# rccohn/AMPIS

Measured on AMD Instinct MI355X. Metric: images/sec Mask R-CNN R50-FPN @1024x1024 inference, higher is better.
Workload: dtype f32 (convs: f16x3 split-operand MFMA -- 22-bit operands, exact products, fp32 accumulate); 1 GPU; BASELINE configs[1]: R50-FPN inference, batch=8 synthetic 1024x1024 micrographs per GPU, K=2, 1000 proposals/img, TEST.DETECTIONS_PER_IMAGE=200, seeded random-init weights, outputs on the host: boxes, scores, classes and every mask as its COCO compressed-RLE counts string (encoded on the device); batch_per_gpu=8, global_batch=8, parallelism=image-parallel replicas x1, no data-path collective

## Files before the change

### ampis_amd/_lib.py

```python
import ctypes as C
import os

_HERE = os.path.dirname(os.path.abspath(__file__))
LIB_PATH = os.path.join(_HERE, "lib", "libampis_hip.so")


class AmpError(RuntimeError):
    pass


class ConvDesc(C.Structure):
    _fields_ = [(n, C.c_int) for n in
                ("B", "H", "W", "Cin", "Cout", "KH", "KW", "stride", "pad", "relu", "res_mode", "out_mode")]


class RpnLevels(C.Structure):
    _fields_ = [("nlevels", C.c_int), ("A", C.c_int), ("ld", C.c_int), ("pred", C.c_void_p * 5),
                ("h", C.c_int * 5), ("w", C.c_int * 5), ("stride", C.c_int * 5), ("anchor_size", C.c_int * 5)]


class FpnFeats(C.Structure):
    _fields_ = [("feat", C.c_void_p * 4), ("h", C.c_int * 4), ("w", C.c_int * 4), ("stride", C.c_int * 4),
                ("C", C.c_int)]

# ... 56 lines not shown

def _declare(L):
    vp, i, f = C.c_void_p, C.c_int, C.c_float
    sig = {
        "amp_version": ([], i),
        "amp_init": ([i, vp, i, C.POINTER(vp)], i),
        "amp_timer_start": ([vp], i),
        "amp_prof_begin": ([vp, i], i),
        "amp_prof_end": ([vp, C.POINTER(ProfSummary)], i),
        "amp_prof_pause": ([vp, i], i),
        "amp_prof_launches": ([vp, C.POINTER(ProfLaunch), i, C.POINTER(i)], i),
        "amp_timer_stop": ([vp, C.POINTER(f)], i),
        "amp_destroy": ([vp], None),
        "amp_sync": ([vp], i),
        "amp_malloc": ([vp, C.c_size_t, C.POINTER(vp)], i),
        "amp_free": ([vp, vp], i),
        "amp_memcpy_h2d": ([vp, vp, vp, C.c_size_t], i),
        "amp_memcpy_d2h": ([vp, vp, vp, C.c_size_t], i),
        "amp_memset": ([vp, vp, i, C.c_size_t], i),
        "amp_conv2d_nhwc": ([vp, C.POINTER(ConvDesc), vp, vp, vp, vp, vp, vp], i),
        "amp_conv2d_nhwc_ex": ([vp, C.POINTER(ConvDesc), vp, vp, vp, vp, vp, vp, vp], i),
        "amp_conv2d_nhwc_fmt": ([vp, C.POINTER(ConvDesc), vp, vp, vp, vp, vp, vp, i], i),
        "amp_unsplit_rows": ([vp, vp, C.c_longlong, i, vp], i),
        "amp_group_expand_weights": ([vp, vp, i, i, i, i, vp], i),
        "amp_resize_scratch_bytes": ([i, i, i, i], C.c_size_t),
        "amp_resize_bilinear_u8": ([vp, vp, i, i, vp, i, i, vp], i),
        "amp_resize_flip_u8": ([vp, vp, i, i, vp, i, i, i, i, vp], i),
        "amp_compact_dets": ([vp, i, i, vp, vp, vp, vp, vp, vp, vp, vp], i),
        "amp_set_conv_mode": ([vp, i], i),
        "amp_get_conv_mode": ([vp], i),
        "amp_conv_range_flag": ([vp, i, C.POINTER(C.c_int)], i),
        "amp_split_weights": ([vp, vp, C.c_longlong, i, vp], i),
        "amp_bottleneck64_tail": ([vp, i, i, i, vp, vp, vp, vp, vp, vp, vp, i, vp, vp], i),
        "amp_conv2d_grouped_nhwc": ([vp, C.POINTER(ConvDesc), i, vp, vp, vp, vp, vp, vp], i),
        "amp_conv2d_grouped_nhwc_fmt": ([vp, C.POINTER(ConvDesc), i, vp, vp, vp, vp, vp, vp, i], i),
        "amp_conv_wgrad_scratch_floats": ([C.POINTER(ConvDesc)], C.c_size_t),
        "amp_conv2d_wgrad": ([vp, C.POINTER(ConvDesc), vp, vp, vp, vp, vp, i], i),
        "amp_conv2d_wgrad_scaled": ([vp, C.POINTER(ConvDesc), vp, vp, vp, vp, vp, i, i, i], i),
        "amp_colsum": ([vp, vp, i, i, vp, vp, i], i),
        "amp_dgrad_weights": ([vp, vp, vp, i, i, i, i, vp], i),
        "amp_dgrad_weights_split": ([vp, vp, vp, i, i, i, i, vp], i),
        "amp_preprocess": ([vp, vp, i, i, i, i, i, C.POINTER(f), C.POINTER(f), vp, vp], i),
        "amp_model_set_image_sizes": ([vp, vp, i], i),
        "amp_maxpool3x3s2": ([vp, vp, i, i, i, i, vp], i),
        "amp_subsample2": ([vp, vp, i, i, i, i, vp], i),
        "amp_rpn_topk": ([vp, C.POINTER(RpnLevels), i, i, vp, i, vp, vp, vp], i),
        "amp_rpn_decode": ([vp, C.POINTER(RpnLevels), i, i, vp, vp, vp, i, i, i, vp, vp, vp], i),
        "amp_rpn_decode_sized": ([vp, C.POINTER(RpnLevels), i, i, vp, vp, vp, i, i, vp, i, vp, vp, vp], i),
        "amp_sort_gather": ([vp, i, i, i, vp, vp, vp, vp, vp, vp, vp, vp, vp], i),
        "amp_sort_gather_n": ([vp, i, i, i, vp, vp, vp, vp, vp, vp, vp, vp, vp, vp], i),
        "amp_nms": ([vp, i, i, vp, vp, vp, f, i, vp, vp, vp], i),
        "amp_rpn_nms_scratch_words": ([i, i, i], C.c_size_t),
        "amp_rpn_nms_levels": ([vp, i, i, i, i, vp, vp, vp, f, i, vp, vp, vp, vp, vp, vp, vp], i),
        "amp_roi_align": ([vp, C.POINTER(FpnFeats), vp, vp, vp, i, i, vp, vp], i),
        "amp_roi_align_fmt": ([vp, C.POINTER(FpnFeats), vp, vp, vp, i, i, vp, vp, i], i),
        "amp_box_candidates": ([vp, vp, i, vp, vp, i, i, i, C.POINTER(f), f, i, i, vp, vp, i, vp, vp], i),
        "amp_box_candidates_sized": ([vp, vp, i, vp, vp, i, i, i, C.POINTER(f), f, i, i, vp, vp, vp, i, vp, vp], i),
        "amp_gather_dets": ([vp, i, i, i, vp, vp, vp, vp, vp, vp, vp, vp, vp, vp], i),
        "amp_mask_prob": ([vp, vp, vp, i, i, vp], i),
        "amp_mask_deconv_predict": ([vp, vp, i, vp, vp, vp, vp, vp, i, vp], i),
        "amp_paste_rle": ([vp, vp, vp, vp, i, vp, vp, i, i, i, f, vp, vp, vp, C.c_ulonglong, vp, vp, vp, vp], i),
        "amp_paste_rle_sized": ([vp, vp, vp, vp, i, vp, vp, i, i, i, vp, f, vp, vp, vp, C.c_ulonglong, vp, vp, vp, vp, vp, C.c_ulonglong, vp], i),
        "amp_rle_to_string": ([vp, i, vp, C.c_size_t, C.POINTER(C.c_size_t)], i),
        "amp_rle_to_strings": ([vp, vp, vp, i, vp, C.c_size_t, vp], i),
        "amp_rle_from_string": ([vp, C.c_size_t, vp, i, C.POINTER(i)], i),
        "amp_rle_encode": ([vp, i, i, vp, i, C.POINTER(i)], i),
# ... 229 lines not shown
```

### ampis_amd/csrc/common.h

```cpp
#pragma once
#include <hip/hip_runtime.h>
#ifdef __HIPCC__
#include <hip/hip_ext.h>
#endif
#include <stdint.h>
#include <stdio.h>
#include <algorithm>
#include <string>

#include "../../include/ampis_hip.h"

namespace amp {

void set_error(const char* fmt, ...);

#define AMP_HIP_CHECK(expr)                                                         \
    do {                                                                            \
        hipError_t _e = (expr);                                                     \
        if (_e != hipSuccess) {                                                     \
            amp::set_error("%s:%d: %s -> %s", __FILE__, __LINE__, #expr,            \
                           hipGetErrorString(_e));                                  \
            return AMP_ERR_HIP;                                                     \
        }                                                                           \
    } while (0)
// ... 140 lines not shown
int comm_mark_producer_end(amp_ctx* ctx);
int comm_wait_done(amp_ctx* ctx);
int comm_agree_flag(amp_ctx* ctx, int* d_flag);
int rle_strings_run(amp_ctx* ctx, const unsigned int* pool, const unsigned long long* off, const int* len, int n, char* str,
                    unsigned long long cap, unsigned long long* str_off, int* str_len, unsigned long long* total);
int roi_align_run(amp_ctx* ctx, const amp_fpn_feats* f, const float* rois, const int* batch_idx, const int* roi_count, int R, int P,
                  float* out, int* level_out, int out_split, int in_split = 0);
int box_candidates_run(amp_ctx* ctx, const float* pred, int ld, const float* proposals, const int* prop_count, int B, int Rcap, int K,
                       const float reg_weights[4], float score_thresh, int img_h, int img_w, const int* img_hw, const float* thresh_img,
                       float* dense_boxes, unsigned long long* keys, int ccap, int* cand_count, int* overflow);
struct WeightJob {
    const float* w;
    const float* scale;
    unsigned int* out;
    int N, KH, KW, C;
    int transpose;
};
int weight_jobs_run(amp_ctx* ctx, const WeightJob* jobs_dev, const void* chunks_dev, int nchunks);
int sgd_chunks_run(amp_ctx* ctx, const unsigned long long* chunks_dev, int nchunks, float* p, const float* g, float* v, float lr,
                   float momentum, float weight_decay, float grad_scale);
int wgrad_async_begin(amp_ctx* ctx, float* scratch1);
int wgrad_async_join(amp_ctx* ctx);
int wgrad_async_end(amp_ctx* ctx);
int roi_align_bwd_run(amp_ctx* ctx, float* const dfeat[4], const int fh[4], const int fw[4], const int stride[4], int C, const float* rois,
                      const int* batch_idx, int R, int P, const float* dout, int B, int init);
int upsample2_bwd_run(amp_ctx* ctx, const float* dfine, float* dcoarse, int B, int Hc, int Wc, int C, int init);
int maxpool_run(amp_ctx* ctx, const float* x, int B, int H, int W, int C, float* y, int y_split);
int compact_dets_run(amp_ctx* ctx, int B, int D, const int* det_count, const float* det_boxes, const float* det_scores, const int* det_classes,
                     float* boxes, float* scores, int* classes, int* batch, int* n_total );
int stem_pool_run(amp_ctx* ctx, int B, int H, int W, const float* x, int x_split, const float* w_split, const float* scale, const float* shift,
                  float* pool, int pool_split);
int conv_c64_fused3_run(amp_ctx* ctx, int B, int H, int W, const float* x_split, const float* w2_split, const float* scale2, const float* shift2,
                        const float* w3_split, const float* scale3, const float* shift3, int C3, const float* res_split, float* y_split);
bool stem_pool_applies(amp_ctx* ctx, const float* w_split);
bool stem_u8_applies(amp_ctx* ctx, const float* w_split);
int stem_pool_u8_run(amp_ctx* ctx, const uint8_t* img, int B, int H, int W, int Hp, int Wp, const float mean[3], const float std_[3],
                     const int* img_hw, const float* w_split, const float* scale, const float* shift, float* pool, int pool_split);
int preprocess_run(amp_ctx* ctx, const uint8_t* img_bgr, int B, int H, int W, int Hp, int Wp, const float mean[3], const float std[3],
                   const int* img_hw, float* out, int out_split);
}
```

### ampis_amd/csrc/conv.hip

```cpp
#include "common.h"
#include <type_traits>

namespace {

typedef float f32x4 __attribute__((ext_vector_type(4)));
typedef float f32x16 __attribute__((ext_vector_type(16)));
typedef _Float16 f16x8 __attribute__((ext_vector_type(8)));
typedef _Float16 f16x2 __attribute__((ext_vector_type(2)));
typedef _Float16 f16x4 __attribute__((ext_vector_type(4)));
typedef unsigned int u32x4 __attribute__((ext_vector_type(4)));
constexpr float LO_SCALE = 2048.0f;

constexpr int BK = 32;
constexpr int LDS_LD = 36;

struct ConvArgs {
    const float* x;
    const float* w;
    const float* scale;
    const float* shift;
    const float* res;
    const float* mask;
    float* y;
    int B, H, W, Cin;
// ... 1903 lines not shown
    const int oyw = oy0 + 4 * wm;
    if constexpr (EPI == 3) {
        const int Ho = a.Ho, Wo = a.Wo, M = a.M;
        conv_epilogue_rpn_rows(a, acc, lds, wave, lane, n0, [=](int i, int r) {
            const int oy = oyw + i, ox = ox0 + r;
            return (oy < Ho && ox < Wo) ? (b * Ho + oy) * Wo + ox : M;
        });
    } else {
#pragma unroll
        for (int h = 0; h < 2; ++h) {
            int mrows[2];
#pragma unroll
            for (int i = 0; i < 2; ++i) {
                const int oy = oyw + 2 * h + i, ox = ox0 + l15;
                mrows[i] = (oy < a.Ho && ox < a.Wo) ? (b * a.Ho + oy) * a.Wo + ox : a.M;
            }
            conv_epilogue_direct_rows<false, true, 2>(a, reinterpret_cast<f32x4 (&)[2][4]>(acc[2 * h]), lane, mrows, n0 + wn * 64);
        }
    }
#ifdef AMP_STAMP
    if (lane == 0)
        for (int q = 0; q < 8; ++q) atomicAdd(&g_stamp[wave * 8 + q], (unsigned long long)st_acc[q]);
#endif
}

struct Fuse3Args {
    const float* w3;
    const float* scale3;
    const float* shift3;
    const float* res;
    float* y;
    int C3;
    unsigned int w3_bytes;
};
template <bool DIAG, bool FUSE3 = false>
__global__ __launch_bounds__(256, 2) void conv3x3_c64_kernel(const ConvArgs a, const unsigned int x_bytes, const unsigned int w_bytes, const int tiles_x, const int tiles_y, const Fuse3Args f3) {
    constexpr int TH = 8, TW = 16, PH = TH + 2, PW = TW + 2, NPIX = PH * PW;
    constexpr int ROWF = 64;
    constexpr int NINST = NPIX / 4;
    static_assert(NPIX % 4 == 0, "patch pixels per DMA instruction");
    __shared__ __attribute__((aligned(16))) float lds[NPIX * ROWF + 2 * 64 * ROWF];
    float* patch = lds;
    float* wbuf = lds + NPIX * ROWF;
    const int tid = threadIdx.x, lane = tid & 63;
    const int wave = __builtin_amdgcn_readfirstlane(tid >> 6);
    const int l15 = lane & 15, lq = lane >> 4;
    int t = amp::xcd_remap(blockIdx.x, a.nblk);
    const int tile_n = t % a.ntn; t /= a.ntn;
    const int tx = t % tiles_x; t /= tiles_x;
    const int ty = t % tiles_y;
    const int b = t / tiles_y;
    const int oy0 = ty * TH, ox0 = tx * TW, n0 = tile_n * 64;
    const int cwin = a.grouped ? n0 : 0;
    const __amdgpu_buffer_rsrc_t rsrc_x = __builtin_amdgcn_make_buffer_rsrc(const_cast<float*>(a.x), 0, x_bytes, 0x00020000);
    const __amdgpu_buffer_rsrc_t rsrc_w = __builtin_amdgcn_make_buffer_rsrc(const_cast<float*>(a.w), 0, w_bytes, 0x00020000);
    const int sub = lane >> 4, chunk = lane & 15;
    for (int it = wave; it < NINST; it += 4) {
        const int q = it * 4 + sub;
        const int py = q / PW, px = q - py * PW;
        const int iy = oy0 - 1 + py, ix = ox0 - 1 + px;
        const bool v = (unsigned)iy < (unsigned)a.H && (unsigned)ix < (unsigned)a.W;
        const unsigned int voff = v ? (unsigned int)((((size_t)(b * a.H + iy) * a.W + ix) * a.Cin + cwin) * 4 + (size_t)((chunk ^ (q & 15)) * 16)) : OOB_VOFF;
        __builtin_amdgcn_raw_ptr_buffer_load_lds(rsrc_x, (__attribute__((address_space(3))) void*)(patch + it * 4 * ROWF), 16, (int)voff, 0, 0, 0);
    }
    auto stage_w = [&](int tap, int buf) {
#pragma unroll
        for (int g = 0; g < 4; ++g) {
            const int r = (wave * 4 + g) * 4 + sub;
            const int n = n0 + swap_channel(r);
            const unsigned int voff = (n < a.Cout) ? (unsigned int)(((size_t)n * a.K + (size_t)tap * 64) * 4 + (size_t)((chunk ^ (r & 15)) * 16)) : OOB_VOFF;
            __builtin_amdgcn_raw_ptr_buffer_load_lds(rsrc_w, (__attribute__((address_space(3))) void*)(wbuf + buf * 64 * ROWF + (wave * 4 + g) * 4 * ROWF), 16, (int)voff, 0, 0, 0);
        }
    };
    stage_w(0, 0);
    f32x4 acc[2][4], acx[2][4];
#pragma unroll
    for (int i = 0; i < 2; ++i)
#pragma unroll
        for (int j = 0; j < 4; ++j)
#pragma unroll
            for (int e = 0; e < 4; ++e) { acc[i][j][e] = 0.f; acx[i][j][e] = 0.f; }
    for (int tap = 0; tap < 9; ++tap) {
        __syncthreads();
        if (tap + 1 < 9) stage_w(tap + 1, (tap + 1) & 1);
        const int ky = tap / 3, kx = tap - 3 * ky;
        const float* wb = wbuf + (tap & 1) * 64 * ROWF;
#pragma unroll
        for (int g = 0; g < 2; ++g) {
            F16x3Frags<2, 4> f;
#pragma unroll
            for (int i = 0; i < 2; ++i) {
                const int q = (2 * wave + i + ky) * PW + kx + l15;
                const float* row = patch + q * ROWF;
                f.ah[i] = *reinterpret_cast<const f16x8*>(row + 4 * ((8 * g + lq) ^ (q & 15)));
                f.al[i] = *reinterpret_cast<const f16x8*>(row + 4 * ((8 * g + 4 + lq) ^ (q & 15)));
            }
            if constexpr (DIAG) {
#pragma unroll
                for (int jj = 0; jj < 2; ++jj) {
                    const float* row = wb + ((2 * g + jj) * 16 + l15) * ROWF;
                    f.bh[jj] = *reinterpret_cast<const f16x8*>(row + 4 * ((8 * g + lq) ^ l15));
                    f.bl[jj] = *reinterpret_cast<const f16x8*>(row + 4 * ((8 * g + 4 + lq) ^ l15));
                }
#pragma unroll
                for (int i = 0; i < 2; ++i) {
#pragma unroll
                    for (int jj = 0; jj < 2; ++jj) acx[i][2 * g + jj] = __builtin_amdgcn_mfma_f32_16x16x32_f16(f.bh[jj], f.al[i], acx[i][2 * g + jj], 0, 0, 0);
#pragma unroll
                    for (int jj = 0; jj < 2; ++jj) acx[i][2 * g + jj] = __builtin_amdgcn_mfma_f32_16x16x32_f16(f.bl[jj], f.ah[i], acx[i][2 * g + jj], 0, 0, 0);
#pragma unroll
                    for (int jj = 0; jj < 2; ++jj) acc[i][2 * g + jj] = __builtin_amdgcn_mfma_f32_16x16x32_f16(f.bh[jj], f.ah[i], acc[i][2 * g + jj], 0, 0, 0);
                }
            } else {
#pragma unroll
                for (int j = 0; j < 4; ++j) {
                    const float* row = wb + (j * 16 + l15) * ROWF;
                    f.bh[j] = *reinterpret_cast<const f16x8*>(row + 4 * ((8 * g + lq) ^ l15));
                    f.bl[j] = *reinterpret_cast<const f16x8*>(row + 4 * ((8 * g + 4 + lq) ^ l15));
                }
                f16x3_mfma16<2, 4, true>(f, acc, acx);
            }
        }
    }
#pragma unroll
    for (int i = 0; i < 2; ++i)
#pragma unroll
        for (int j = 0; j < 4; ++j)
#pragma unroll
            for (int e = 0; e < 4; ++e) acc[i][j][e] = __fadd_rn(acc[i][j][e], __fmul_rn(acx[i][j][e], 1.0f / LO_SCALE));
    int mrows[2];
#pragma unroll
    for (int i = 0; i < 2; ++i) {
        const int oy = oy0 + 2 * wave + i, ox = ox0 + l15;
        mrows[i] = (oy < a.Ho && ox < a.Wo) ? (b * a.Ho + oy) * a.Wo + ox : a.M;
    }
    if constexpr (!FUSE3) {
        conv_epilogue_direct_rows<false, true, 2>(a, acc, lane, mrows, n0);
    } else {
        f16x8 t2h[2][2], t2l[2][2];
        f32x2 chk = {0.f, 0.f};
#pragma unroll
        for (int g = 0; g < 2; ++g) {
            f32x2 sc[4], sh[4];
            const int n = 32 * g + 8 * lq;
#pragma unroll
            for (int p = 0; p < 4; ++p) {
                sc[p] = a.scale ? f32x2{a.scale[n + 2 * p], a.scale[n + 2 * p + 1]} : f32x2{1.f, 1.f};
                sh[p] = a.shift ? f32x2{a.shift[n + 2 * p], a.shift[n + 2 * p + 1]} : f32x2{0.f, 0.f};
            }
#pragma unroll
            for (int i = 0; i < 2; ++i) {
#pragma unroll
                for (int p = 0; p < 4; ++p) {
                    const f32x4& blk = acc[i][2 * g + (p >> 1)];
                    const f32x2 v = {blk[2 * (p & 1)], blk[2 * (p & 1) + 1]};
                    chk = __builtin_elementwise_fma(v, f32x2{0.f, 0.f}, chk);
                    f32x2 o = v * sc[p] + sh[p];
                    if (a.relu) { o[0] = fmaxf(o[0], 0.f); o[1] = fmaxf(o[1], 0.f); }
                    const f16x2 h = __builtin_convertvector(o, f16x2);
                    const f32x2 hf = {(float)h[0], (float)h[1]};
                    const f32x2 l = __builtin_elementwise_fma(hf, f32x2{-LO_SCALE, -LO_SCALE}, o * LO_SCALE);
                    const f16x2 lh = __builtin_convertvector(l, f16x2);
                    t2h[i][g][2 * p] = h[0]; t2h[i][g][2 * p + 1] = h[1];
                    t2l[i][g][2 * p] = lh[0]; t2l[i][g][2 * p + 1] = lh[1];
                }
            }
        }
        if (!(chk[0] == 0.f) || !(chk[1] == 0.f)) atomicOr(a.range_flag, 1);
        __syncthreads();
        const __amdgpu_buffer_rsrc_t rsrc_w3 = __builtin_amdgcn_make_buffer_rsrc(const_cast<float*>(f3.w3), 0, f3.w3_bytes, 0x00020000);
        float* w3s = lds;
        const int ninst3 = f3.C3 / 4;
        for (int it = wave; it < ninst3; it += 4) {
            const int r = it * 4 + sub;
            const int n = (r & ~63) + swap_channel(r & 63);
            const unsigned int voff = (unsigned int)((size_t)n * 256 + (size_t)((chunk ^ (r & 15)) * 16));
            __builtin_amdgcn_raw_ptr_buffer_load_lds(rsrc_w3, (__attribute__((address_space(3))) void*)(w3s + it * 4 * ROWF), 16, (int)voff, 0, 0, 0);
        }
        __syncthreads();
        ConvArgs a3 = a;
        a3.scale = f3.scale3; a3.shift = f3.shift3; a3.res = f3.res; a3.mask = nullptr; a3.y = f3.y;
        a3.Cout = f3.C3; a3.relu = 1; a3.res_mode = 1; a3.res_split = 1; a3.y_split = 1; a3.out_mode = 0; a3.mask_split = 0;
        for (int c = 0; c < f3.C3 / 64; ++c) {
            f32x4 acc3[2][4], acx3[2][4];
#pragma unroll
            for (int i = 0; i < 2; ++i)
#pragma unroll
                for (int j = 0; j < 4; ++j)
#pragma unroll
                    for (int e = 0; e < 4; ++e) { acc3[i][j][e] = 0.f; acx3[i][j][e] = 0.f; }
            const float* wc = w3s + c * 64 * ROWF;
#pragma unroll
            for (int g = 0; g < 2; ++g) {
                F16x3Frags<2, 4> f;
#pragma unroll
                for (int i = 0; i < 2; ++i) { f.ah[i] = t2h[i][g]; f.al[i] = t2l[i][g]; }
#pragma unroll
                for (int j = 0; j < 4; ++j) {
                    const float* row = wc + (j * 16 + l15) * ROWF;
                    f.bh[j] = *reinterpret_cast<const f16x8*>(row + 4 * ((8 * g + lq) ^ l15));
// ... 1275 lines not shown
    if (C3 % 64 != 0 || C3 > 256 || B < 1 || H < 1 || W < 1) return 1;
    const size_t x_bytes = (size_t)B * H * W * 64 * sizeof(float), w_bytes = (size_t)64 * 576 * sizeof(float), r_bytes = (size_t)B * H * W * C3 * sizeof(float);
    const long long tiles = (long long)B * amp::cdiv(H, 8) * amp::cdiv(W, 16);
    if (x_bytes >= (size_t)OOB_VOFF || r_bytes >= ((size_t)1 << 32) || (long long)B * H * W >= (1ll << 29) / 4 || (g_patch_conv != 2 && tiles < 512)) return 1;
    ConvArgs a = ConvArgs();
    a.x = x_split; a.w = w2_split; a.scale = scale2; a.shift = shift2;
    a.B = B; a.H = H; a.W = W; a.Cin = 64; a.Cout = 64; a.KH = 3; a.KW = 3; a.stride = 1; a.pad = 1; a.Ho = H; a.Wo = W;
    a.M = B * H * W; a.K = 576; a.nsteps = 18; a.cin_win = 64; a.grouped = 0;
    a.relu = 1; a.in_scale = a.out_scale = 1.0f; a.y_split = 1; a.direct_epi = 1;
    a.range_flag = ctx->d_conv_flag;
    a.ntn = 1; a.nblk = (int)tiles;
    set_fastdiv((unsigned int)(a.Ho * a.Wo), &a.div_howo_mul, &a.div_howo_shr);
    set_fastdiv((unsigned int)a.Wo, &a.div_wo_mul, &a.div_wo_shr);
    Fuse3Args f3;
    f3.w3 = w3_split; f3.scale3 = scale3; f3.shift3 = shift3; f3.res = res_split; f3.y = y_split; f3.C3 = C3; f3.w3_bytes = (unsigned int)((size_t)C3 * 64 * sizeof(float));
    amp_prof_rec* rec = nullptr;
    if (ctx->prof_on) {
        if (ctx->prof_used < ctx->prof_pool.size()) {
            rec = &ctx->prof_pool[ctx->prof_used++];
            rec->flops = 2.0 * (double)a.M * (64.0 * 576.0 + (double)C3 * 64.0);
            rec->variant = 1;
            rec->bytes = (double)x_bytes + (double)w_bytes + (double)f3.w3_bytes + 2.0 * (double)r_bytes;
            rec->M = a.M; rec->N = C3; rec->K = 576 + 64;
        } else {
            ctx->prof_truncated = true;
        }
    }
    amp::ProfLaunchScope timed(rec ? rec->e0 : nullptr, rec ? rec->e1 : nullptr);
    AMP_TIMED_LAUNCH((conv3x3_c64_kernel<false, true>), dim3(a.nblk), dim3(256), 0, ctx->stream, a, (unsigned int)x_bytes, (unsigned int)w_bytes, amp::cdiv(W, 16), amp::cdiv(H, 8), f3);
    AMP_HIP_CHECK(hipGetLastError());
    return AMP_OK;
}

extern "C" int amp_bottleneck64_tail(amp_ctx* ctx, int B, int H, int W, const float* x_split, const float* w2_split, const float* scale2, const float* shift2,
                                     const float* w3_split, const float* scale3, const float* shift3, int C3, const float* res_split, float* y_split) {
    AMP_REQUIRE(ctx && x_split && w2_split && w3_split && res_split && y_split, "%s", "amp_bottleneck64_tail: null argument");
    const int st = amp::conv_c64_fused3_run(ctx, B, H, W, x_split, w2_split, scale2, shift2, w3_split, scale3, shift3, C3, res_split, y_split);
    if (st == 1) { amp::set_error("amp_bottleneck64_tail: the fused kernel does not apply (AMP_CONV_F16X3, C3 %% 64 == 0, C3 <= 256, >= 512 tiles of 8 x 16)"); return AMP_ERR_STATE; }
    return st;
}
```

### ampis_amd/csrc/model.hip

```cpp
#include <math.h>
#include <string.h>

#include <map>
#include <string>
#include <vector>

#include "common.h"

namespace {

struct ConvW {
    float* w = nullptr;
    float* scale = nullptr;
    float* shift = nullptr;
    int cout = 0, cin = 0, kh = 0, kw = 0;
    float* w_split = nullptr;
    float* wt_split = nullptr;
    float w_absmax = 0.f;
    int groups = 1;
};

struct NamedBuf {
    void* ptr;
    int dtype;
// ... 297 lines not shown
        if (fused < 0) return fused;
        if (fused == 1 && x0_split) { amp::set_error("amp_model: the input was split for the fused stem, which then did not launch"); return AMP_ERR_STATE; }
        if (fused == 1) {
            AMP_TRY(launch_conv(m, sw, x0, B, Hp, Wp, 2, 3, true, 0, nullptr, 0, stem));
            AMP_TRY(amp::maxpool_run(ctx, stem, B, h, w, 64, pool, native_all ? 1 : 0));
        }
    }
    if (!dry) tap(m, "stem_pool", pool, native_all ? SPL : 0, {B, h4, w4, 64});

    float* cur = pool;
    int ch = h4, cw_ = w4;
    float* res_out[4];
    int res_h[4], res_w[4];
    for (int s = 0; s < 4; ++s) {
        for (int b = 0; b < m->nblk[s]; ++b) {
            const std::string p = std::string("backbone.bottom_up.") + kStage[s] + "." + std::to_string(b);
            const int st = (b == 0) ? kStride[s] : 1;
            const int oh = (ch - 1) / st + 1, ow = (cw_ - 1) / st + 1;
            const size_t mark = ws.off;
            AMP_ALLOC(out, float, (size_t)B * oh * ow * kOut[s]);
            const size_t keep = ws.off;
            const float* shortcut = cur;
            if (b == 0) {
                AMP_ALLOC(sc, float, (size_t)B * oh * ow * kOut[s]);
                if (!dry) AMP_TRY(launch_conv(m, CONV((p + ".shortcut").c_str()), cur, B, ch, cw_, st, 0, false, 0, nullptr, 0, sc, FMT(native_all, native_all, false)));
                shortcut = sc;
            }
            const int st1 = c.stride_in_1x1 ? st : 1, st2 = c.stride_in_1x1 ? 1 : st;
            const int h1 = (ch - 1) / st1 + 1, w1 = (cw_ - 1) / st1 + 1;
            AMP_ALLOC(t1, float, (size_t)B * h1 * w1 * m->mid[s]);
            AMP_ALLOC(t2, float, (size_t)B * oh * ow * m->mid[s]);
            if (!dry) {
                const bool t1s = reads_split(p + ".conv2"), t2s = reads_split(p + ".conv3");
                AMP_TRY(launch_conv(m, CONV((p + ".conv1").c_str()), cur, B, ch, cw_, st1, 0, true, 0, nullptr, 0, t1, FMT(native_all, t1s, false)));
                int fused23 = 1;
                const ConvW &c2w = CONV((p + ".conv2").c_str()), &c3w = CONV((p + ".conv3").c_str());
                if (s == 0 && t1s && t2s && native_all && st2 == 1 && c2w.groups == 1 && c2w.cin == 64 && c2w.cout == 64 && c2w.kh == 3 && c3w.cin == 64 && c3w.kh == 1 &&
                    !m->split_stale && c2w.scale && c3w.scale)
                    fused23 = amp::conv_c64_fused3_run(ctx, B, oh, ow, t1, c2w.w_split, c2w.scale, c2w.shift, c3w.w_split, c3w.scale, c3w.shift, c3w.cout, shortcut, out);
                if (fused23 < 0) return fused23;
                if (fused23 == 1) {
                    AMP_TRY(launch_conv(m, c2w, t1, B, h1, w1, st2, 1, true, 0, nullptr, 0, t2, FMT(t1s, t2s, false)));
                    AMP_TRY(launch_conv(m, c3w, t2, B, oh, ow, 1, 0, true, 1, shortcut, 0, out, FMT(t2s, native_all, native_all)));
                }
            }
            (void)mark;
            if (m->saving) {
                amp_model::BlockAct ba;
                ba.key = p; ba.x_in = cur; ba.t1 = t1; ba.t2 = t2; ba.sc = (b == 0) ? const_cast<float*>(shortcut) : nullptr; ba.out = out;
                ba.in_h = ch; ba.in_w = cw_; ba.oh = oh; ba.ow = ow; ba.cin = (b == 0) ? (s == 0 ? 64 : kOut[s - 1]) : kOut[s];
                ba.mid = m->mid[s]; ba.cout = kOut[s]; ba.stride = st; ba.stage = s; ba.has_sc = (b == 0);
                if (!dry) m->blocks.push_back(ba);
            } else {
                ws.off = keep;
            }
            cur = out;
            ch = oh; cw_ = ow;
        }
        res_out[s] = cur; res_h[s] = ch; res_w[s] = cw_;
        if (!dry) tap(m, kStage[s], cur, native_all ? SPL : 0, {B, ch, cw_, kOut[s]});
    }

    float* feat[5];
    int fh[5], fw[5];
    const int fstride[5] = {4, 8, 16, 32, 64};
    float* prev_lat = nullptr;
    for (int l = 5; l >= 2; --l) {
        const int s = l - 2;
        const std::string ln = "backbone.fpn_lateral" + std::to_string(l), on = "backbone.fpn_output" + std::to_string(l);
        AMP_ALLOC(lat, float, (size_t)B * res_h[s] * res_w[s] * 256);
        AMP_ALLOC(outp, float, (size_t)B * res_h[s] * res_w[s] * 256);
        if (!dry) {
// ... 1913 lines not shown
```

### ampis_amd/ops.py

```python
import ctypes as C

import torch

from . import _lib
from ._lib import ConvDesc, check, lib, ptr


def torch_context(device=0):
    if not torch.cuda.is_available():
        raise _lib.AmpError("no HIP device visible: the ampis_amd hot path has no CPU fallback")
    with torch.cuda.device(device):
        return _lib.Context(device, borrow_stream=torch.cuda.current_stream().cuda_stream)


def _f32c(t):
    assert t is None or (t.is_cuda and t.dtype == torch.float32 and t.is_contiguous()), "need contiguous fp32 CUDA tensor"
    return t


FMT_X_SPLIT, FMT_Y_SPLIT, FMT_RES_SPLIT = 1, 2, 4


def split_rows(ctx, t):
    _f32c(t)
# ... 19 lines not shown
    Wo = (W + 2 * pad - KW) // stride + 1
    if res_mode is None:
        res_mode = 0 if res is None else 1
    d = ConvDesc(B, H, W, Cin, Cout, KH, KW, stride, pad, int(relu), int(res_mode), 2 if scatter2 else int(deconv2x2))
    if out is not None:
        y = out
    elif deconv2x2:
        y = torch.empty((B, 2 * Ho, 2 * Wo, Cout // 4), device=x.device, dtype=torch.float32)
    elif scatter2:
        y = torch.zeros((B, 2 * Ho, 2 * Wo, Cout), device=x.device, dtype=torch.float32)
    else:
        y = torch.empty((B, Ho, Wo, Cout), device=x.device, dtype=torch.float32)
    if fmt:
        assert mask is None
        check(lib().amp_conv2d_nhwc_fmt(ctx.handle, C.byref(d), ptr(x), ptr(w), ptr(scale), ptr(shift), ptr(res), ptr(y), int(fmt)),
              "amp_conv2d_nhwc_fmt")
        return y
    check(lib().amp_conv2d_nhwc_ex(ctx.handle, C.byref(d), ptr(x), ptr(w), ptr(scale), ptr(shift), ptr(res), ptr(_f32c(mask)), ptr(y)),
          "amp_conv2d_nhwc_ex")
    return y


def bottleneck64_tail(ctx, x_split, w2, scale2, shift2, w3, scale3, shift3, res_split):
    _f32c(x_split), _f32c(w2), _f32c(w3), _f32c(res_split)
    B, H, W, _ = x_split.shape
    C3 = w3.shape[0]
    w2s, w3s = split_rows(ctx, w2.reshape(64, 576)), split_rows(ctx, w3.reshape(C3, 64))
    y = torch.empty((B, H, W, C3), device=x_split.device, dtype=torch.float32)
    check(lib().amp_bottleneck64_tail(ctx.handle, B, H, W, ptr(x_split), ptr(w2s), ptr(_f32c(scale2)), ptr(_f32c(shift2)), ptr(w3s), ptr(_f32c(scale3)),
                                      ptr(_f32c(shift3)), C3, ptr(res_split), ptr(y)), "amp_bottleneck64_tail")
    return y


def conv2d_grouped_nhwc(ctx, x, w, groups, scale=None, shift=None, res=None, stride=1, pad=0, relu=False, fmt=0):
    _f32c(x), _f32c(w), _f32c(scale), _f32c(shift), _f32c(res)
    B, H, W, Cin = x.shape
    Cout, KH, KW, cpg = w.shape
    assert Cin == Cout and cpg * groups == Cin
    w_win = torch.empty((Cout, KH, KW, 64), device=x.device, dtype=torch.float32)
    check(lib().amp_group_expand_weights(ctx.handle, ptr(w), Cout, KH, KW, cpg, ptr(w_win)), "amp_group_expand_weights")
    Ho = (H + 2 * pad - KH) // stride + 1
    Wo = (W + 2 * pad - KW) // stride + 1
    d = ConvDesc(B, H, W, Cin, Cout, KH, KW, stride, pad, int(relu), 0 if res is None else 1, 0)
    y = torch.empty((B, Ho, Wo, Cout), device=x.device, dtype=torch.float32)
    if fmt:
        check(lib().amp_conv2d_grouped_nhwc_fmt(ctx.handle, C.byref(d), int(groups), ptr(x), ptr(w_win), ptr(scale), ptr(shift), ptr(res), ptr(y), int(fmt)),
              "amp_conv2d_grouped_nhwc_fmt")
        return y
    check(lib().amp_conv2d_grouped_nhwc(ctx.handle, C.byref(d), int(groups), ptr(x), ptr(w_win), ptr(scale), ptr(shift), ptr(res), ptr(y)),
          "amp_conv2d_grouped_nhwc")
    return y


def resize_bilinear_u8(ctx, img, h, w):
    import numpy as np
    img = np.ascontiguousarray(img, dtype=np.uint8)
    H, W, _ = img.shape
    src = torch.from_numpy(img).to("cuda:%d" % ctx.device)
    dst = torch.empty((h, w, 3), dtype=torch.uint8, device=src.device)
    tmp = torch.empty(int(lib().amp_resize_scratch_bytes(H, W, h, w)), dtype=torch.uint8, device=src.device)
    torch.cuda.synchronize()
    check(lib().amp_resize_bilinear_u8(ctx.handle, ptr(src), H, W, ptr(dst), h, w, ptr(tmp)), "amp_resize_bilinear_u8")
    check(lib().amp_sync(ctx.handle), "amp_sync")
    return dst.cpu().numpy()


# ... 200 lines not shown
```

### include/ampis_hip.h

```cpp
#ifndef AMPIS_HIP_H
#define AMPIS_HIP_H

#include <stddef.h>
#include <stdint.h>

#ifdef __cplusplus
extern "C" {
#endif

typedef enum amp_status {
    AMP_OK = 0,
    AMP_ERR_ARG = -1,
    AMP_ERR_HIP = -2,
    AMP_ERR_NOMEM = -3,
    AMP_ERR_STATE = -4
} amp_status;

typedef struct amp_ctx amp_ctx;

const char* amp_last_error(void);
int  amp_version(void);
#define AMP_STREAM_BORROW 1
int  amp_init(int device, void* hip_stream, int flags, amp_ctx** out);
void amp_destroy(amp_ctx* ctx);
// ... 35 lines not shown
int amp_resize_bilinear_u8(amp_ctx* ctx, const unsigned char* src, int H, int W, unsigned char* dst, int h, int w, void* tmp);
int amp_resize_flip_u8(amp_ctx* ctx, const unsigned char* src, int H, int W, unsigned char* dst, int dst_pitch, int h, int w, int flip, void* tmp);

typedef struct amp_conv_desc {
    int B, H, W, Cin;
    int Cout;
    int KH, KW, stride, pad;
    int relu;
    int res_mode;
    int out_mode;
} amp_conv_desc;
int amp_conv2d_nhwc(amp_ctx* ctx, const amp_conv_desc* d, const float* x, const float* w,
                    const float* scale, const float* shift, const float* res, float* y);
int amp_group_expand_weights(amp_ctx* ctx, const float* w, int Cout, int KH, int KW, int cpg, float* w_win);
int amp_conv2d_grouped_nhwc(amp_ctx* ctx, const amp_conv_desc* d, int groups, const float* x, const float* w_win,
                            const float* scale, const float* shift, const float* res, float* y);
int amp_conv2d_grouped_nhwc_fmt(amp_ctx* ctx, const amp_conv_desc* d, int groups, const float* x, const float* w_win,
                                const float* scale, const float* shift, const float* res, float* y, int fmt);
size_t amp_grouped_wgrad_scratch_floats(const amp_conv_desc* d);
int amp_conv2d_grouped_wgrad(amp_ctx* ctx, const amp_conv_desc* d, int groups, const float* x, const float* dy, const float* scale,
                             float* scratch, float* grad_win);
int amp_conv2d_grouped_wgrad_fmt(amp_ctx* ctx, const amp_conv_desc* d, int groups, const float* x, const float* dy, const float* scale,
                                 float* scratch, float* grad_win, int fmt, int dy_shift);
int amp_group_dgrad_weights(amp_ctx* ctx, const float* w_win, const float* scale, int C, int KH, int KW, float* wt_win);
int amp_conv2d_nhwc_ex(amp_ctx* ctx, const amp_conv_desc* d, const float* x, const float* w, const float* scale, const float* shift,
                       const float* res, const float* mask, float* y);

enum { AMP_FMT_X_SPLIT = 1, AMP_FMT_Y_SPLIT = 2, AMP_FMT_RES_SPLIT = 4, AMP_FMT_MASK_SPLIT = 8 };
int amp_conv2d_nhwc_fmt(amp_ctx* ctx, const amp_conv_desc* d, const float* x, const float* w, const float* scale, const float* shift,
                        const float* res, float* y, int fmt);
int amp_unsplit_rows(amp_ctx* ctx, const float* x_split, long long rows, int C, float* out);
int amp_bottleneck64_tail(amp_ctx* ctx, int B, int H, int W, const float* x_split, const float* w2_split, const float* scale2, const float* shift2,
                          const float* w3_split, const float* scale3, const float* shift3, int C3, const float* res_split, float* y_split);

size_t amp_conv_wgrad_scratch_floats(const amp_conv_desc* d);
int amp_conv2d_wgrad(amp_ctx* ctx, const amp_conv_desc* d, const float* x, const float* dy, const float* scale, float* scratch,
                     float* grad, int accumulate);
int amp_conv2d_wgrad_scaled(amp_ctx* ctx, const amp_conv_desc* d, const float* x, const float* dy, const float* scale, float* scratch,
                            float* grad, int accumulate, int dy_shift, int x_shift);
int amp_conv2d_wgrad_fmt(amp_ctx* ctx, const amp_conv_desc* d, const float* x, const float* dy, const float* scale, float* scratch,
                            float* grad, int accumulate, int dy_shift, int x_shift, int x_split, float* bias_grad, int bias_accumulate);
int amp_colsum(amp_ctx* ctx, const float* dy, int M, int N, float* scratch, float* out, int accumulate);
int amp_colsum_split(amp_ctx* ctx, const float* dy, int M, int N, float* scratch, float* out, int accumulate, float* dy_split, int shift);
int amp_colsum_of_split(amp_ctx* ctx, const float* dy_split, int M, int N, float* scratch, float* out, int accumulate, int shift);
int amp_dgrad_weights(amp_ctx* ctx, const float* w, const float* scale, int Cout, int KH, int KW, int Cin, float* wt);
int amp_dgrad_weights_split(amp_ctx* ctx, const float* w, const float* scale, int Cout, int KH, int KW, int Cin, float* wt_split);
int amp_roi_align_bwd(amp_ctx* ctx, float* const dfeat[4], const int fh[4], const int fw[4], const int stride[4], int C, const float* rois,
                      const int* batch_idx, int R, int P, const float* dout);
int amp_roi_align_bwd_batched(amp_ctx* ctx, float* const dfeat[4], const int fh[4], const int fw[4], const int stride[4], int C, const float* rois,
                              const int* batch_idx, int R, int P, const float* dout, int B);
int amp_upsample2_bwd(amp_ctx* ctx, const float* dfine, float* dcoarse, int B, int Hc, int Wc, int C);
int amp_subsample2_bwd(amp_ctx* ctx, const float* dy, float* dx, int B, int H, int W, int C);
int amp_relu_mask(amp_ctx* ctx, float* g, const float* act, size_t n);
int amp_relu_mask_split(amp_ctx* ctx, float* g, const float* act_split, size_t n, int C);
int amp_relu_mask_to_split(amp_ctx* ctx, const float* g, const float* act_split, float* out_split, size_t n, int C, int shift);
int amp_subsample2_bwd_split(amp_ctx* ctx, const float* dy_split, float* dx, int B, int H, int W, int C, int shift);
int amp_accumulate_split(amp_ctx* ctx, const float* dy_split, float* dx, long long rows, int C, int shift);
int amp_scatter2_rows(amp_ctx* ctx, const float* src, float* up, int B, int H, int W, int C);
int amp_small_k_dgrad(amp_ctx* ctx, const float* dl, int ld, int K, const float* w, int C, const float* act, float* dx, size_t npix);
int amp_small_k_dgrad_split(amp_ctx* ctx, const float* dl, int K, const float* w, int C, const float* act_split, float* dx_split, int npix,
                            int shift, float* scratch, float* colsum_out, int accumulate);
int amp_small_k_dgrad_split_f32act(amp_ctx* ctx, const float* dl, int ld, int K, const float* w, int C, const float* act, float* dx_split, int npix,
                                   int shift, float* scratch, float* colsum_out, int accumulate);
int amp_small_k_dgrad_split_ld(amp_ctx* ctx, const float* dl, int ld, int K, const float* w, int C, const float* act_split, float* dx_split, int npix,
                               int shift, float* scratch, float* colsum_out, int accumulate);
int amp_colsum_finish(amp_ctx* ctx, const float* partial, int parts, int N, float* out, int accumulate);
// ... 234 lines not shown
```

Before: 517.8 images/s.

## Fuse conv1 1x1 into the conv2+conv3 bottleneck kernel for stage-1 blocks

Adds a whole-bottleneck kernel variant for the 64-channel res2 stage. It computes the 1x1 conv1 over the halo patch in registers, writes the split f16 result into LDS, and then runs the existing fused 3x3 + 1x1 tail. This removes the t1 intermediate's global write and read and one kernel launch per block. In exchange, conv1 is recomputed on halo pixels (10x18 patch for an 8x16 tile), which adds FLOPs, and register pressure rises from the extra accumulators.

```diff
diff --git a/ampis_amd/_lib.py b/ampis_amd/_lib.py
--- a/ampis_amd/_lib.py
+++ b/ampis_amd/_lib.py
@@ -112,6 +112,7 @@
         "amp_conv_range_flag": ([vp, i, C.POINTER(C.c_int)], i),
         "amp_split_weights": ([vp, vp, C.c_longlong, i, vp], i),
         "amp_bottleneck64_tail": ([vp, i, i, i, vp, vp, vp, vp, vp, vp, vp, i, vp, vp], i),
+        "amp_bottleneck64_block": ([vp, i, i, i, i, vp, vp, vp, vp, vp, vp, vp, vp, vp, vp, i, vp, vp], i),
         "amp_conv2d_grouped_nhwc": ([vp, C.POINTER(ConvDesc), i, vp, vp, vp, vp, vp, vp], i),
         "amp_conv2d_grouped_nhwc_fmt": ([vp, C.POINTER(ConvDesc), i, vp, vp, vp, vp, vp, vp, i], i),
         "amp_conv_wgrad_scratch_floats": ([C.POINTER(ConvDesc)], C.c_size_t),
diff --git a/ampis_amd/csrc/common.h b/ampis_amd/csrc/common.h
--- a/ampis_amd/csrc/common.h
+++ b/ampis_amd/csrc/common.h
@@ -196,6 +196,9 @@
                   float* pool, int pool_split);
 int conv_c64_fused3_run(amp_ctx* ctx, int B, int H, int W, const float* x_split, const float* w2_split, const float* scale2, const float* shift2,
                         const float* w3_split, const float* scale3, const float* shift3, int C3, const float* res_split, float* y_split);
+int conv_c64_block_run(amp_ctx* ctx, int B, int H, int W, int Cin1, const float* x_split, const float* w1_split, const float* scale1, const float* shift1,
+                       const float* w2_split, const float* scale2, const float* shift2, const float* w3_split, const float* scale3, const float* shift3, int C3,
+                       const float* res_split, float* y_split);
 bool stem_pool_applies(amp_ctx* ctx, const float* w_split);
 bool stem_u8_applies(amp_ctx* ctx, const float* w_split);
 int stem_pool_u8_run(amp_ctx* ctx, const uint8_t* img, int B, int H, int W, int Hp, int Wp, const float mean[3], const float std_[3],
diff --git a/ampis_amd/csrc/conv.hip b/ampis_amd/csrc/conv.hip
--- a/ampis_amd/csrc/conv.hip
+++ b/ampis_amd/csrc/conv.hip
@@ -1959,9 +1959,49 @@
     float* y;
     int C3;
     unsigned int w3_bytes;
+    const float* x1;
+    const float* w1;
+    const float* scale1;
+    const float* shift1;
+    int Cin1;
+    unsigned int x1_bytes, w1_bytes;
 };
-template <bool DIAG, bool FUSE3 = false>
+
+template <int MB>
+__device__ __forceinline__ void epilogue_split_regs(const f32x4 (&acc)[MB][4], const float* scale, const float* shift, bool relu, int nw0, int lq,
+                                                    f16x8 (&th)[MB][2], f16x8 (&tl)[MB][2], f32x2& chk) {
+#pragma unroll
+    for (int g = 0; g < 2; ++g) {
+        f32x2 sc[4], sh[4];
+        const int n = nw0 + 32 * g + 8 * lq;
+#pragma unroll
+        for (int p = 0; p < 4; ++p) {
+            sc[p] = scale ? f32x2{scale[n + 2 * p], scale[n + 2 * p + 1]} : f32x2{1.f, 1.f};
+            sh[p] = shift ? f32x2{shift[n + 2 * p], shift[n + 2 * p + 1]} : f32x2{0.f, 0.f};
+        }
+#pragma unroll
+        for (int i = 0; i < MB; ++i) {
+#pragma unroll
+            for (int p = 0; p < 4; ++p) {
+                const f32x4& blk = acc[i][2 * g + (p >> 1)];
+                const f32x2 v = {blk[2 * (p & 1)], blk[2 * (p & 1) + 1]};
+                chk = __builtin_elementwise_fma(v, f32x2{0.f, 0.f}, chk);
+                f32x2 o = v * sc[p] + sh[p];
+                if (relu) { o[0] = fmaxf(o[0], 0.f); o[1] = fmaxf(o[1], 0.f); }
+                const f16x2 h = __builtin_convertvector(o, f16x2);
+                const f32x2 hf = {(float)h[0], (float)h[1]};
+                const f32x2 l = __builtin_elementwise_fma(hf, f32x2{-LO_SCALE, -LO_SCALE}, o * LO_SCALE);
+                const f16x2 lh = __builtin_convertvector(l, f16x2);
+                th[i][g][2 * p] = h[0]; th[i][g][2 * p + 1] = h[1];
+                tl[i][g][2 * p] = lh[0]; tl[i][g][2 * p + 1] = lh[1];
+            }
+        }
+    }
+}
+
+template <bool DIAG, bool FUSE3 = false, bool BLOCK = false>
 __global__ __launch_bounds__(256, 2) void conv3x3_c64_kernel(const ConvArgs a, const unsigned int x_bytes, const unsigned int w_bytes, const int tiles_x, const int tiles_y, const Fuse3Args f3) {
+    static_assert(!BLOCK || (FUSE3 && !DIAG), "the whole-block kernel extends the fused conv2 + conv3 one");
     constexpr int TH = 8, TW = 16, PH = TH + 2, PW = TW + 2, NPIX = PH * PW;
     constexpr int ROWF = 64;
     constexpr int NINST = NPIX / 4;
@@ -1982,14 +2022,16 @@
     const __amdgpu_buffer_rsrc_t rsrc_x = __builtin_amdgcn_make_buffer_rsrc(const_cast<float*>(a.x), 0, x_bytes, 0x00020000);
     const __amdgpu_buffer_rsrc_t rsrc_w = __builtin_amdgcn_make_buffer_rsrc(const_cast<float*>(a.w), 0, w_bytes, 0x00020000);
     const int sub = lane >> 4, chunk = lane & 15;
-    for (int it = wave; it < NINST; it += 4) {
-        const int q = it * 4 + sub;
-        const int py = q / PW, px = q - py * PW;
-        const int iy = oy0 - 1 + py, ix = ox0 - 1 + px;
-        const bool v = (unsigned)iy < (unsigned)a.H && (unsigned)ix < (unsigned)a.W;
-        const unsigned int voff = v ? (unsigned int)((((size_t)(b * a.H + iy) * a.W + ix) * a.Cin + cwin) * 4 + (size_t)((chunk ^ (q & 15)) * 16)) : OOB_VOFF;
-        __builtin_amdgcn_raw_ptr_buffer_load_lds(rsrc_x, (__attribute__((address_space(3))) void*)(patch + it * 4 * ROWF), 16, (int)voff, 0, 0, 0);
-    }
+    auto stage_patch = [&](const __amdgpu_buffer_rsrc_t rs, int cin, int c0) {
+        for (int it = wave; it < NINST; it += 4) {
+            const int q = it * 4 + sub;
+            const int py = q / PW, px = q - py * PW;
+            const int iy = oy0 - 1 + py, ix = ox0 - 1 + px;
+            const bool v = (unsigned)iy < (unsigned)a.H && (unsigned)ix < (unsigned)a.W;
+            const unsigned int voff = v ? (unsigned int)((((size_t)(b * a.H + iy) * a.W + ix) * cin + c0) * 4 + (size_t)((chunk ^ (q & 15)) * 16)) : OOB_VOFF;
+            __builtin_amdgcn_raw_ptr_buffer_load_lds(rs, (__attribute__((address_space(3))) void*)(patch + it * 4 * ROWF), 16, (int)voff, 0, 0, 0);
+        }
+    };
     auto stage_w = [&](int tap, int buf) {
 #pragma unroll
         for (int g = 0; g < 4; ++g) {
@@ -1999,7 +2041,81 @@
             __builtin_amdgcn_raw_ptr_buffer_load_lds(rsrc_w, (__attribute__((address_space(3))) void*)(wbuf + buf * 64 * ROWF + (wave * 4 + g) * 4 * ROWF), 16, (int)voff, 0, 0, 0);
         }
     };
-    stage_w(0, 0);
+    if constexpr (!BLOCK) {
+        stage_patch(rsrc_x, a.Cin, cwin);
+        stage_w(0, 0);
+    } else {
+        const __amdgpu_buffer_rsrc_t rsrc_x1 = __builtin_amdgcn_make_buffer_rsrc(const_cast<float*>(f3.x1), 0, f3.x1_bytes, 0x00020000);
+        const __amdgpu_buffer_rsrc_t rsrc_w1 = __builtin_amdgcn_make_buffer_rsrc(const_cast<float*>(f3.w1), 0, f3.w1_bytes, 0x00020000);
+        float* w1buf = wbuf + 64 * ROWF;
+        stage_w(0, 0);
+        f32x4 acc1[3][4], acx1[3][4];
+#pragma unroll
+        for (int i = 0; i < 3; ++i)
+#pragma unroll
+            for (int j = 0; j < 4; ++j)
+#pragma unroll
+                for (int e = 0; e < 4; ++e) { acc1[i][j][e] = 0.f; acx1[i][j][e] = 0.f; }
+        int q1[3];
+#pragma unroll
+        for (int i = 0; i < 3; ++i) q1[i] = min(16 * (3 * wave + i) + l15, NPIX - 1);
+        const int nk = f3.Cin1 / 64;
+        for (int k = 0; k < nk; ++k) {
+            if (k > 0) __syncthreads();
+            stage_patch(rsrc_x1, f3.Cin1, 64 * k);
+#pragma unroll
+            for (int g = 0; g < 4; ++g) {
+                const int r = (wave * 4 + g) * 4 + sub;
+                const unsigned int voff = (unsigned int)(((size_t)swap_channel(r) * f3.Cin1 + (size_t)k * 64) * 4 + (size_t)((chunk ^ (r & 15)) * 16));
+                __builtin_amdgcn_raw_ptr_buffer_load_lds(rsrc_w1, (__attribute__((address_space(3))) void*)(w1buf + (wave * 4 + g) * 4 * ROWF), 16, (int)voff, 0, 0, 0);
+            }
+            __syncthreads();
+#pragma unroll
+            for (int g = 0; g < 2; ++g) {
+                F16x3Frags<3, 4> f;
+#pragma unroll
+                for (int i = 0; i < 3; ++i) {
+                    const float* row = patch + q1[i] * ROWF;
+                    f.ah[i] = *reinterpret_cast<const f16x8*>(row + 4 * ((8 * g + lq) ^ (q1[i] & 15)));
+                    f.al[i] = *reinterpret_cast<const f16x8*>(row + 4 * ((8 * g + 4 + lq) ^ (q1[i] & 15)));
+                }
+#pragma unroll
+                for (int j = 0; j < 4; ++j) {
+                    const float* row = w1buf + (j * 16 + l15) * ROWF;
+                    f.bh[j] = *reinterpret_cast<const f16x8*>(row + 4 * ((8 * g + lq) ^ l15));
+                    f.bl[j] = *reinterpret_cast<const f16x8*>(row + 4 * ((8 * g + 4 + lq) ^ l15));
+                }
+                f16x3_mfma16<3, 4, true>(f, acc1, acx1);
+            }
+        }
+#pragma unroll
+        for (int i = 0; i < 3; ++i)
+#pragma unroll
+            for (int j = 0; j < 4; ++j)
+#pragma unroll
+                for (int e = 0; e < 4; ++e) acc1[i][j][e] = __fadd_rn(acc1[i][j][e], __fmul_rn(acx1[i][j][e], 1.0f / LO_SCALE));
+        f16x8 t1h[3][2], t1l[3][2];
+        f32x2 chk1 = {0.f, 0.f};
+        epilogue_split_regs<3>(acc1, f3.scale1, f3.shift1, true, 0, lq, t1h, t1l, chk1);
+        if (!(chk1[0] == 0.f) || !(chk1[1] == 0.f)) atomicOr(a.range_flag, 1);
+        __syncthreads();
+#pragma unroll
+        for (int i = 0; i < 3; ++i) {
+            const int q = 16 * (3 * wave + i) + l15;
+            const int py = q / PW, px = q - py * PW;
+            const int iy = oy0 - 1 + py, ix = ox0 - 1 + px;
+            const bool inside = (unsigned)iy < (unsigned)a.H && (unsigned)ix < (unsigned)a.W;
+            if (q < NPIX) {
+                float* row = patch + q * ROWF;
+                const f16x8 z = {};
+#pragma unroll
+                for (int g = 0; g < 2; ++g) {
+                    *reinterpret_cast<f16x8*>(row + 4 * ((8 * g + lq) ^ (q & 15))) = inside ? t1h[i][g] : z;
+                    *reinterpret_cast<f16x8*>(row + 4 * ((8 * g + 4 + lq) ^ (q & 15))) = inside ? t1l[i][g] : z;
+                }
+            }
+        }
+    }
     f32x4 acc[2][4], acx[2][4];
 #pragma unroll
     for (int i = 0; i < 2; ++i)
@@ -2066,33 +2182,7 @@
     } else {
         f16x8 t2h[2][2], t2l[2][2];
         f32x2 chk = {0.f, 0.f};
-#pragma unroll
-        for (int g = 0; g < 2; ++g) {
-            f32x2 sc[4], sh[4];
-            const int n = 32 * g + 8 * lq;
-#pragma unroll
-            for (int p = 0; p < 4; ++p) {
-                sc[p] = a.scale ? f32x2{a.scale[n + 2 * p], a.scale[n + 2 * p + 1]} : f32x2{1.f, 1.f};
-                sh[p] = a.shift ? f32x2{a.shift[n + 2 * p], a.shift[n + 2 * p + 1]} : f32x2{0.f, 0.f};
-            }
-#pragma unroll
-            for (int i = 0; i < 2; ++i) {
-#pragma unroll
-                for (int p = 0; p < 4; ++p) {
-                    const f32x4& blk = acc[i][2 * g + (p >> 1)];
-                    const f32x2 v = {blk[2 * (p & 1)], blk[2 * (p & 1) + 1]};
-                    chk = __builtin_elementwise_fma(v, f32x2{0.f, 0.f}, chk);
-                    f32x2 o = v * sc[p] + sh[p];
-                    if (a.relu) { o[0] = fmaxf(o[0], 0.f); o[1] = fmaxf(o[1], 0.f); }
-                    const f16x2 h = __builtin_convertvector(o, f16x2);
-                    const f32x2 hf = {(float)h[0], (float)h[1]};
-                    const f32x2 l = __builtin_elementwise_fma(hf, f32x2{-LO_SCALE, -LO_SCALE}, o * LO_SCALE);
-                    const f16x2 lh = __builtin_convertvector(l, f16x2);
-                    t2h[i][g][2 * p] = h[0]; t2h[i][g][2 * p + 1] = h[1];
-                    t2l[i][g][2 * p] = lh[0]; t2l[i][g][2 * p + 1] = lh[1];
-                }
-            }
-        }
+        epilogue_split_regs<2>(acc, a.scale, a.shift, a.relu != 0, 0, lq, t2h, t2l, chk);
         if (!(chk[0] == 0.f) || !(chk[1] == 0.f)) atomicOr(a.range_flag, 1);
         __syncthreads();
         const __amdgpu_buffer_rsrc_t rsrc_w3 = __builtin_amdgcn_make_buffer_rsrc(const_cast<float*>(f3.w3), 0, f3.w3_bytes, 0x00020000);
@@ -3434,6 +3524,63 @@
     return AMP_OK;
 }
 
+static int g_fuse_block = getenv("AMP_NO_FUSE_BLOCK") ? 0 : 1;
+extern "C" void amp_debug_set_fuse_block(int v) { g_fuse_block = v; }
+int amp::conv_c64_block_run(amp_ctx* ctx, int B, int H, int W, int Cin1, const float* x_split, const float* w1_split, const float* scale1, const float* shift1,
+                            const float* w2_split, const float* scale2, const float* shift2, const float* w3_split, const float* scale3, const float* shift3, int C3,
+                            const float* res_split, float* y_split) {
+    if (!g_fuse_block || !g_fuse23 || g_patch_conv == 0 || !g_direct_epi || ctx->conv_mode != AMP_CONV_F16X3 || !w1_split || !w2_split || !w3_split) return 1;
+    if (C3 % 64 != 0 || C3 > 256 || Cin1 % 64 != 0 || Cin1 < 64 || Cin1 > 1024 || B < 1 || H < 1 || W < 1) return 1;
+    const size_t M = (size_t)B * H * W;
+    const size_t x1_bytes = M * Cin1 * sizeof(float), w_bytes = (size_t)64 * 576 * sizeof(float), r_bytes = M * C3 * sizeof(float);
+    const long long tiles = (long long)B * amp::cdiv(H, 8) * amp::cdiv(W, 16);
+    if (x1_bytes >= (size_t)OOB_VOFF || r_bytes >= ((size_t)1 << 32) || (long long)M >= (1ll << 29) / 4 || (g_patch_conv != 2 && tiles < 512)) return 1;
+    ConvArgs a = ConvArgs();
+    a.x = x_split; a.w = w2_split; a.scale = scale2; a.shift = shift2;
+    a.B = B; a.H = H; a.W = W; a.Cin = 64; a.Cout = 64; a.KH = 3; a.KW = 3; a.stride = 1; a.pad = 1; a.Ho = H; a.Wo = W;
+    a.M = (int)M; a.K = 576; a.nsteps = 18; a.cin_win = 64; a.grouped = 0;
+    a.relu = 1; a.in_scale = a.out_scale = 1.0f; a.y_split = 1; a.direct_epi = 1;
+    a.range_flag = ctx->d_conv_flag;
+    a.ntn = 1; a.nblk = (int)tiles;
+    set_fastdiv((unsigned int)(a.Ho * a.Wo), &a.div_howo_mul, &a.div_howo_shr);
+    set_fastdiv((unsigned int)a.Wo, &a.div_wo_mul, &a.div_wo_shr);
+    Fuse3Args f3 = Fuse3Args();
+    f3.w3 = w3_split; f3.scale3 = scale3; f3.shift3 = shift3; f3.res = res_split; f3.y = y_split; f3.C3 = C3;
+    f3.w3_bytes = (unsigned int)((size_t)C3 * 64 * sizeof(float));
+    f3.x1 = x_split; f3.w1 = w1_split; f3.scale1 = scale1; f3.shift1 = shift1; f3.Cin1 = Cin1;
+    f3.x1_bytes = (unsigned int)x1_bytes; f3.w1_bytes = (unsigned int)((size_t)64 * Cin1 * sizeof(float));
+    amp_prof_rec* rec = nullptr;
+    if (ctx->prof_on) {
+        if (ctx->prof_used < ctx->prof_pool.size()) {
+            rec = &ctx->prof_pool[ctx->prof_used++];
+            rec->flops = 2.0 * (double)M * (64.0 * Cin1 + 64.0 * 576.0 + (double)C3 * 64.0);
+            rec->variant = 1;
+            rec->bytes = (double)x1_bytes + (double)f3.w1_bytes + (double)w_bytes + (double)f3.w3_bytes + 2.0 * (double)r_bytes;
+            rec->M = a.M; rec->N = C3; rec->K = Cin1 + 576 + 64;
+        } else {
+            ctx->prof_truncated = true;
+        }
+    }
+    amp::ProfLaunchScope timed(rec ? rec->e0 : nullptr, rec ? rec->e1 : nullptr);
+    AMP_TIMED_LAUNCH((conv3x3_c64_kernel<false, true, true>), dim3(a.nblk), dim3(256), 0, ctx->stream, a, (unsigned int)x1_bytes, (unsigned int)w_bytes, amp::cdiv(W, 16), amp::cdiv(H, 8), f3);
+    AMP_HIP_CHECK(hipGetLastError());
+    return AMP_OK;
+}
+
+extern "C" int amp_bottleneck64_block(amp_ctx* ctx, int B, int H, int W, int Cin1, const float* x_split, const float* w1_split, const float* scale1, const float* shift1,
+                                      const float* w2_split, const float* scale2, const float* shift2, const float* w3_split, const float* scale3, const float* shift3, int C3,
+                                      const float* res_split, float* y_split) {
+    AMP_REQUIRE(ctx && x_split && w1_split && w2_split && w3_split && res_split && y_split, "%s", "amp_bottleneck64_block: null argument");
+    const int st = amp::conv_c64_block_run(ctx, B, H, W, Cin1, x_split, w1_split, scale1, shift1, w2_split, scale2, shift2, w3_split, scale3, shift3, C3,
+                                           res_split, y_split);
+    if (st == 1) {
+        amp::set_error("amp_bottleneck64_block: the fused kernel does not apply (AMP_CONV_F16X3, C3 %% 64 == 0, C3 <= 256, Cin1 %% 64 == 0, Cin1 <= 1024, "
+                       ">= 512 tiles of 8 x 16)");
+        return AMP_ERR_STATE;
+    }
+    return st;
+}
+
 extern "C" int amp_bottleneck64_tail(amp_ctx* ctx, int B, int H, int W, const float* x_split, const float* w2_split, const float* scale2, const float* shift2,
                                      const float* w3_split, const float* scale3, const float* shift3, int C3, const float* res_split, float* y_split) {
     AMP_REQUIRE(ctx && x_split && w2_split && w3_split && res_split && y_split, "%s", "amp_bottleneck64_tail: null argument");
diff --git a/ampis_amd/csrc/model.hip b/ampis_amd/csrc/model.hip
--- a/ampis_amd/csrc/model.hip
+++ b/ampis_amd/csrc/model.hip
@@ -353,12 +353,20 @@
             AMP_ALLOC(t2, float, (size_t)B * oh * ow * m->mid[s]);
             if (!dry) {
                 const bool t1s = reads_split(p + ".conv2"), t2s = reads_split(p + ".conv3");
-                AMP_TRY(launch_conv(m, CONV((p + ".conv1").c_str()), cur, B, ch, cw_, st1, 0, true, 0, nullptr, 0, t1, FMT(native_all, t1s, false)));
-                int fused23 = 1;
-                const ConvW &c2w = CONV((p + ".conv2").c_str()), &c3w = CONV((p + ".conv3").c_str());
-                if (s == 0 && t1s && t2s && native_all && st2 == 1 && c2w.groups == 1 && c2w.cin == 64 && c2w.cout == 64 && c2w.kh == 3 && c3w.cin == 64 && c3w.kh == 1 &&
-                    !m->split_stale && c2w.scale && c3w.scale)
-                    fused23 = amp::conv_c64_fused3_run(ctx, B, oh, ow, t1, c2w.w_split, c2w.scale, c2w.shift, c3w.w_split, c3w.scale, c3w.shift, c3w.cout, shortcut, out);
+                const ConvW &c1w = CONV((p + ".conv1").c_str()), &c2w = CONV((p + ".conv2").c_str()), &c3w = CONV((p + ".conv3").c_str());
+                const bool tail_ok = s == 0 && t1s && t2s && native_all && st2 == 1 && c2w.groups == 1 && c2w.cin == 64 && c2w.cout == 64 && c2w.kh == 3 && c3w.cin == 64 &&
+                                     c3w.kh == 1 && !m->split_stale && c2w.scale && c3w.scale;
+                int fused_block = 1;
+                if (tail_ok && st1 == 1 && c1w.groups == 1 && c1w.kh == 1 && c1w.kw == 1 && c1w.cout == 64 && c1w.scale)
+                    fused_block = amp::conv_c64_block_run(ctx, B, oh, ow, c1w.cin, cur, c1w.w_split, c1w.scale, c1w.shift, c2w.w_split, c2w.scale, c2w.shift,
+                                                          c3w.w_split, c3w.scale, c3w.shift, c3w.cout, shortcut, out);
+                if (fused_block < 0) return fused_block;
+                int fused23 = fused_block == 1 ? 1 : 0;
+                if (fused_block == 1) {
+                    AMP_TRY(launch_conv(m, c1w, cur, B, ch, cw_, st1, 0, true, 0, nullptr, 0, t1, FMT(native_all, t1s, false)));
+                    if (tail_ok)
+                        fused23 = amp::conv_c64_fused3_run(ctx, B, oh, ow, t1, c2w.w_split, c2w.scale, c2w.shift, c3w.w_split, c3w.scale, c3w.shift, c3w.cout, shortcut, out);
+                }
                 if (fused23 < 0) return fused23;
                 if (fused23 == 1) {
                     AMP_TRY(launch_conv(m, c2w, t1, B, h1, w1, st2, 1, true, 0, nullptr, 0, t2, FMT(t1s, t2s, false)));
diff --git a/ampis_amd/ops.py b/ampis_amd/ops.py
--- a/ampis_amd/ops.py
+++ b/ampis_amd/ops.py
@@ -75,6 +75,18 @@
     return y
 
 
+def bottleneck64_block(ctx, x_split, w1, scale1, shift1, w2, scale2, shift2, w3, scale3, shift3, res_split=None):
+    _f32c(x_split), _f32c(w1), _f32c(w2), _f32c(w3), _f32c(res_split)
+    B, H, W, Cin1 = x_split.shape
+    C3 = w3.shape[0]
+    res = x_split if res_split is None else res_split
+    w1s, w2s, w3s = split_rows(ctx, w1.reshape(64, Cin1)), split_rows(ctx, w2.reshape(64, 576)), split_rows(ctx, w3.reshape(C3, 64))
+    y = torch.empty((B, H, W, C3), device=x_split.device, dtype=torch.float32)
+    check(lib().amp_bottleneck64_block(ctx.handle, B, H, W, Cin1, ptr(x_split), ptr(w1s), ptr(_f32c(scale1)), ptr(_f32c(shift1)), ptr(w2s),
+                                       ptr(_f32c(scale2)), ptr(_f32c(shift2)), ptr(w3s), ptr(_f32c(scale3)), ptr(_f32c(shift3)), C3, ptr(res), ptr(y)),
+          "amp_bottleneck64_block")
+    return y
+
 def conv2d_grouped_nhwc(ctx, x, w, groups, scale=None, shift=None, res=None, stride=1, pad=0, relu=False, fmt=0):
     _f32c(x), _f32c(w), _f32c(scale), _f32c(shift), _f32c(res)
     B, H, W, Cin = x.shape
diff --git a/include/ampis_hip.h b/include/ampis_hip.h
--- a/include/ampis_hip.h
+++ b/include/ampis_hip.h
@@ -91,6 +91,9 @@
 int amp_unsplit_rows(amp_ctx* ctx, const float* x_split, long long rows, int C, float* out);
 int amp_bottleneck64_tail(amp_ctx* ctx, int B, int H, int W, const float* x_split, const float* w2_split, const float* scale2, const float* shift2,
                           const float* w3_split, const float* scale3, const float* shift3, int C3, const float* res_split, float* y_split);
+int amp_bottleneck64_block(amp_ctx* ctx, int B, int H, int W, int Cin1, const float* x_split, const float* w1_split, const float* scale1, const float* shift1,
+                           const float* w2_split, const float* scale2, const float* shift2, const float* w3_split, const float* scale3, const float* shift3, int C3,
+                           const float* res_split, float* y_split);
 
 size_t amp_conv_wgrad_scratch_floats(const amp_conv_desc* d);
 int amp_conv2d_wgrad(amp_ctx* ctx, const amp_conv_desc* d, const float* x, const float* dy, const float* scale, float* scratch,
```

Measured after the change: 523.1 images/s, median of 6. No clear change (+1.0%).
